# shamim-hussain/tgt

Hardware: AMD Instinct MI355X
Metric: graphs/sec training step, TGT-At 24L PCQM batch 256, 1/2/4/8 MI355X (higher is better)
Workload: dtype bf16

## Files before the change

tgt_amd/csrc/triplet_attention_bwd2.hip:

```cpp
#include <cstdlib>
#include "triplet_common.hpp"

namespace tgt {
namespace bwd2 {

typedef short s16x4 __attribute__((ext_vector_type(4)));
typedef __attribute__((address_space(3))) s16x4 lds_s16x4;

constexpr int HG = 8, D = 16, kThreads = 512;
constexpr int kRow = 256;
constexpr int kSlab = 32 * kRow;
constexpr int kSet = 4 * kSlab;
constexpr int kXch = 2 * 2048;
template <bool DMA> struct Lay {
#ifndef TGT_BWD2_DEPTH
#define TGT_BWD2_DEPTH 2
#endif
    static constexpr int kDepth = TGT_BWD2_DEPTH;
    static constexpr int kSets = DMA ? kDepth + 1 : 2;
    static constexpr int kOffXch = kSets * kSet;
    static constexpr int kOffPart = kOffXch + HG * kXch;
    static constexpr int kLds = kOffPart;
};
typedef __attribute__((address_space(3))) void lds_void;
#if TGT_LD_AUX == 2
#define TGT_BWD2_LD_POLICY " nt"
#else
#define TGT_BWD2_LD_POLICY ""
#endif

__device__ __forceinline__ int swz(int row) { return ((row & 7) << 1) | ((row >> 3) & 1); }
__device__ __forceinline__ int slab_off(int row, int cb) { return row * kRow + ((((cb >> 4) ^ swz(row)) & 15) << 4) + (cb & 15); }

__device__ __forceinline__ s16x4 tr_read(uint32_t addr) {
    return __builtin_amdgcn_ds_read_tr16_b64_v4i16(reinterpret_cast<lds_s16x4*>(addr));
}
template <typename T>
__device__ __forceinline__ frag_t<T> frag_of(s16x4 lo, s16x4 hi) {
    frag_t<T> f;
    __builtin_memcpy(&f, &lo, 8);
    __builtin_memcpy(reinterpret_cast<char*>(&f) + 8, &hi, 8);
    return f;
}
__device__ __forceinline__ f32x4 mma16(bf16x8 a, bf16x8 b, f32x4 c) { return __builtin_amdgcn_mfma_f32_16x16x32_bf16(a, b, c, 0, 0, 0); }
__device__ __forceinline__ f32x4 mma16(f16x8 a, f16x8 b, f32x4 c) { return __builtin_amdgcn_mfma_f32_16x16x32_f16(a, b, c, 0, 0, 0); }

template <typename T> struct Vec4;
template <> struct Vec4<bf16_t> { typedef __attribute__((ext_vector_type(4))) __bf16 type; };
template <> struct Vec4<f16_t> { typedef __attribute__((ext_vector_type(4))) _Float16 type; };
template <typename T>
__device__ __forceinline__ uint2 pack4(float a, float b, float c, float d) {
    typename Vec4<T>::type t;
    t[0] = from_f32<T>(a); t[1] = from_f32<T>(b); t[2] = from_f32<T>(c); t[3] = from_f32<T>(d);
    uint2 v;
    __builtin_memcpy(&v, &t, 8);
    return v;
}
template <typename T>
__device__ __forceinline__ uint2 frag_half(const frag_t<T>& f, int h) {
    uint2 v;
    __builtin_memcpy(&v, reinterpret_cast<const char*>(&f) + 8 * h, 8);
    return v;
}

template <typename T>
__device__ __forceinline__ void arm_load16(const ThirdArm& ta, int b, int dir, int g, int N, char* lds, int tid) {
    using A = ArmStage<T, HG, 1>;
    const int pitch = A::pitch(dir), mpitch = A::mpitch(dir);
    const char* eg = reinterpret_cast<const char*>(ta.eg);
    for (int idx = tid; idx < 32 * 32 * 2; idx += kThreads) {
        const int half = idx & 1, pr = idx >> 1, yy = pr & 31, xx = pr >> 5;
        uint4 v = make_uint4(0, 0, 0, 0);
        if (xx < N && yy < N && (half == 0 ? ta.biased : ta.gated))
            v = *reinterpret_cast<const uint4*>(eg + ((((int64_t)b * N + xx) * N + yy) * ta.ld + (half == 0 ? ta.e_off : ta.g_off) + g * HG) * 2);
        uint32_t* dst = reinterpret_cast<uint32_t*>(lds + xx * pitch + yy * A::kPairBytes + half * 16);
        dst[0] = v.x; dst[1] = v.y; dst[2] = v.z; dst[3] = v.w;
    }
    for (int idx = tid; idx < 32 * 32; idx += kThreads) {
        const int yy = idx & 31, xx = idx >> 5;
        float m = 0.f;
        if (xx < N && yy < N && ta.mask) m = ta.mask[((int64_t)b * N + xx) * N + yy];
        *reinterpret_cast<float*>(lds + A::kOffM + xx * mpitch + yy * 4) = m;
    }
}
template <typename T>
__device__ __forceinline__ void arm_store16(const ThirdArm& ta, void* d_eg, int b, int dir, int g, int N, const char* lds, int tid,
                                            float (&sums)[HG]) {
    using A = ArmStage<T, HG, 1>;
    const int pitch = A::pitch(dir);
    char* deg = reinterpret_cast<char*>(d_eg);
    static_assert(kThreads % 2 == 0, "a thread must own one piece (E or G)");
#pragma nounroll
    for (int idx = tid; idx < 32 * 32 * 2; idx += kThreads) {
        const int half = idx & 1, pr = idx >> 1, yy = pr & 31, xx = pr >> 5;
        if (xx < N && yy < N && (half == 0 ? ta.biased : ta.gated)) {
            const uint32_t* src = reinterpret_cast<const uint32_t*>(lds + xx * pitch + yy * A::kPairBytes + half * 16);
            const uint4 v = make_uint4(src[0], src[1], src[2], src[3]);
            *reinterpret_cast<uint4*>(deg + ((((int64_t)b * N + xx) * N + yy) * ta.ld + (half == 0 ? ta.e_off : ta.g_off) + g * HG) * 2) = v;
            T t[HG];
            __builtin_memcpy(t, &v, 16);
#pragma unroll
            for (int h = 0; h < HG; ++h) sums[h] += to_f32(t[h]);
        }
    }
}

__device__ __forceinline__ void zero_grad_rows(__amdgpu_buffer_rsrc_t r_grd, uint32_t wQ, uint32_t wK, uint32_t qo, uint32_t ko, uint32_t vo,
                                               uint32_t gQj, uint32_t gKj, int j0, int N) {
    const u32x4_t z = {0, 0, 0, 0};
    for (int j = j0; j < N; ++j) {
        __builtin_amdgcn_raw_buffer_store_b128(z, r_grd, (int)wQ, (int)(qo + (uint32_t)j * gQj), TGT_ST_AUX);
        __builtin_amdgcn_raw_buffer_store_b128(z, r_grd, (int)wK, (int)(ko + (uint32_t)j * gKj), TGT_ST_AUX);
        __builtin_amdgcn_raw_buffer_store_b128(z, r_grd, (int)wK, (int)(vo + (uint32_t)j * gKj), TGT_ST_AUX);
    }
}

template <typename T, bool CS, int FL, bool DMA, typename... NC>
__global__ void __launch_bounds__(kThreads, 2) __attribute__((amdgpu_waves_per_eu(2, 2))) tri_att_bwd2_kernel(const tgt_triplet_attention_args a, NC... nc) {
    constexpr bool RG = sizeof...(NC) > 0;
    const int32_t* node_counts = tri_counts_ptr(nc...);
    using F = frag_t<T>;
    constexpr int kOffXch = Lay<DMA>::kOffXch, kOffPart = Lay<DMA>::kOffPart;
    using G = TriGeo<T, D, HG>;
    extern __shared__ __attribute__((aligned(16))) char smem[];
    const uint32_t sbase = (uint32_t)(uintptr_t)smem;

    const int tid = threadIdx.x, lane = tid & 63, wave = tid >> 6;
    const int r = lane & 31, hi = lane >> 5;
    const int p16 = lane & 15, g16 = lane >> 4;
    const TriCtx c = tri_ctx<T, D, HG>(a, wave);
    const int N = c.N;
    const ThirdArm ta = tri_third_arm(a, c.dir);
    const bool biased = FL >= 0 ? (FL & TGT_TRI_BIASED) != 0 : ta.biased, gated = FL >= 0 ? (FL & TGT_TRI_GATED) != 0 : ta.gated;
    constexpr float kLog2e = 1.4426950408889634f;
    const float scale2 = a.scale * kLog2e;
#ifdef TGT_PROBES
    const int ablate = a._pad0;
#else
    constexpr int ablate = 0;
#endif

    const int64_t Nl = N;
    const int64_t ldq = a.ld_dqkv[c.dir] ? a.ld_dqkv[c.dir] : a.ld_qkv[c.dir];
    const int64_t lde = a.ld_deg[c.dir] ? a.ld_deg[c.dir] : a.ld_eg[c.dir];
    const uint32_t hch = (uint32_t)(c.g * HG * D * 2);
    const uint32_t lds_ = (uint32_t)(a.ld_qkv[c.dir] * 2), ldg_ = (uint32_t)(ldq * 2), ldo_ = (uint32_t)(a.ld_out * 2);
    const __amdgpu_buffer_rsrc_t r_src = graph_rsrc(a.qkv[c.dir], Nl * Nl * a.ld_qkv[c.dir] * 2, c.b);
    const __amdgpu_buffer_rsrc_t r_grd = graph_rsrc(a.d_qkv[c.dir], Nl * Nl * ldq * 2, c.b);
    const __amdgpu_buffer_rsrc_t r_do = graph_rsrc(a.d_out, Nl * Nl * a.ld_out * 2, c.b);
    const __amdgpu_buffer_rsrc_t r_src0 = __builtin_amdgcn_make_buffer_rsrc(const_cast<void*>(a.qkv[c.dir]), 0, 0, 0x00020000);
    const __amdgpu_buffer_rsrc_t r_do0 = __builtin_amdgcn_make_buffer_rsrc(const_cast<void*>(a.d_out), 0, 0, 0x00020000);
    const uint32_t qo = (uint32_t)(a.q_off[c.dir] * 2) + hch, ko = (uint32_t)(a.k_off[c.dir] * 2) + hch, vo = (uint32_t)(a.v_off[c.dir] * 2) + hch;
    const uint32_t oo = (uint32_t)(a.o_off[c.dir] * 2) + hch;
    const bool inward = c.dir == 0;
#ifdef TGT_PROBES
    const bool contig = (ablate & 8) != 0;
#else
    constexpr bool contig = false;
#endif
    const uint32_t sQr = contig ? lds_ : (uint32_t)N * lds_, sQj = contig ? (uint32_t)N * lds_ : lds_;
    const uint32_t sKr = (inward || contig) ? lds_ : (uint32_t)N * lds_, sKj = (inward || contig) ? (uint32_t)N * lds_ : lds_;
    const uint32_t gQr = contig ? ldg_ : (uint32_t)N * ldg_, gQj = contig ? (uint32_t)N * ldg_ : ldg_;
    const uint32_t gKr = (inward || contig) ? ldg_ : (uint32_t)N * ldg_, gKj = (inward || contig) ? (uint32_t)N * ldg_ : ldg_;
    const uint32_t oQr = contig ? ldo_ : (uint32_t)N * ldo_, oQj = contig ? (uint32_t)N * ldo_ : ldo_;
    ThirdArm dta = ta;
    dta.ld = lde;

    const int crow = tid >> 4, cslot = tid & 15;
    const uint32_t lslot16 = (uint32_t)((cslot ^ swz(crow)) & 15) * 16u;
    const uint32_t kOOB = 0x80000000u;
    const bool rowok = crow < N;
    const uint32_t vQ = rowok ? (uint32_t)crow * sQr + lslot16 : kOOB;
    const uint32_t vK = rowok ? (uint32_t)crow * sKr + lslot16 : kOOB;
    const uint32_t vO = rowok ? (uint32_t)crow * oQr + lslot16 : kOOB;
    const uint32_t wQ = rowok ? (uint32_t)crow * gQr + lslot16 : kOOB;
    const uint32_t wK = rowok ? (uint32_t)crow * gKr + lslot16 : kOOB;
    const int chunk = crow * kRow + cslot * 16;

    float* part = reinterpret_cast<float*>(smem + kOffXch);

    const bool dead = a.graph_scale && a.graph_scale[c.b] == 0.f;
    if (dead) {
        zero_grad_rows(r_grd, wQ, wK, qo, ko, vo, gQj, gKj, 0, N);
        const float zero16[16] = {0.f, 0.f, 0.f, 0.f, 0.f, 0.f, 0.f, 0.f, 0.f, 0.f, 0.f, 0.f, 0.f, 0.f, 0.f, 0.f};
        arm_stage_put_grad<T, HG, 1>(smem, c.dir, wave, r, hi, 0, zero16, zero16);
        __syncthreads();
        float unused[HG] = {0.f, 0.f, 0.f, 0.f, 0.f, 0.f, 0.f, 0.f};
        arm_store16<T>(dta, a.d_eg[c.dir], c.b, c.dir, c.g, N, smem, tid, unused);
        if constexpr (CS) {
            float* row = a.d_qkv_colsum[c.dir] + (int64_t)c.b * ldq + c.g * HG * D;
            if (tid < HG * D) {
                row[a.q_off[c.dir] + tid] = 0.f;
                row[a.k_off[c.dir] + tid] = 0.f;
                row[a.v_off[c.dir] + tid] = 0.f;
            }
            if (tid < 2 * HG && (biased || gated)) {
                float* erow = a.d_eg_colsum[c.dir] + (int64_t)c.b * lde;
                if (tid < HG) { if (biased) erow[a.e_off[c.dir] + c.g * HG + tid] = 0.f; }
                else if (gated) erow[a.g_off[c.dir] + c.g * HG + tid - HG] = 0.f;
            }
        }
        return;
    }

    const int n = tri_node_count<RG>(node_counts, c.b, N);
    if constexpr (RG) zero_grad_rows(r_grd, wQ, wK, qo, ko, vo, gQj, gKj, n, N);
    f32x2 biasM[8], gate[8], dE[8], dG[8];
    arm_load16<T>(ta, c.b, c.dir, c.g, N, smem, tid);
    __syncthreads();
    {
        float b16[16], g16[16];
        arm_stage_read<T, HG, 1, true>(ta, smem, c.dir, wave, N, r, hi, 0, 0, b16, g16);
#pragma unroll
        for (int q = 0; q < 16; ++q) {
            const float bl = b16[q] * kLog2e;
            b16[q] = (bl == -INFINITY && b16[q] != -INFINITY) ? -3.402823466e38f : bl;
        }
#pragma unroll
        for (int k = 0; k < 8; ++k) {
            biasM[k] = f32x2{b16[2 * k], b16[2 * k + 1]};
            gate[k] = f32x2{g16[2 * k], g16[2 * k + 1]};
            dE[k] = dG[k] = f32x2{0.f, 0.f};
        }
    }
    __syncthreads();

    const int hb = wave * 32;
    const uint32_t a_frag = (uint32_t)slab_off(r, hb + 16 * hi);
    const int c2 = p16 & 3, pr = p16 >> 2;
    const uint32_t a_kt0 = (uint32_t)slab_off(4 * hi + pr, hb + 8 * c2);
    const uint32_t a_kt1 = (uint32_t)slab_off(8 + 4 * hi + pr, hb + 8 * c2);
    const uint32_t a_qt = (uint32_t)slab_off(4 * g16 + pr, hb + 8 * c2);
    const uint32_t xw = (uint32_t)(kOffXch + wave * kXch + r * 32 + ((hi ^ ((r >> 2) & 3)) << 3));
    const uint32_t xr = (uint32_t)(kOffXch + wave * kXch + (4 * g16 + pr) * 32 + ((c2 ^ g16) << 3));
    const uint32_t w_q = (uint32_t)slab_off(r, hb + 8 * hi);
    const uint32_t w_kv = (uint32_t)slab_off(p16, hb + 8 * g16);

    f32x2 csq[4], csk[2], csv[2];
    if constexpr (CS) {
#pragma unroll
        for (int k = 0; k < 4; ++k) csq[k] = f32x2{0.f, 0.f};
        csk[0] = csk[1] = csv[0] = csv[1] = f32x2{0.f, 0.f};
    }

    auto issue = [&](u32x4_t (&pre)[4], int jj) {
        const bool live = jj < n && !(ablate & 1);
        const __amdgpu_buffer_rsrc_t rs = live ? r_src : r_src0, ro = live ? r_do : r_do0;
        pre[0] = __builtin_amdgcn_raw_buffer_load_b128(rs, (int)vQ, (int)(qo + (uint32_t)jj * sQj), TGT_LD_AUX);
        pre[1] = __builtin_amdgcn_raw_buffer_load_b128(ro, (int)vO, (int)(oo + (uint32_t)jj * oQj), TGT_LD_AUX);
        pre[2] = __builtin_amdgcn_raw_buffer_load_b128(rs, (int)vK, (int)(ko + (uint32_t)jj * sKj), TGT_LD_AUX);
        pre[3] = __builtin_amdgcn_raw_buffer_load_b128(rs, (int)vK, (int)(vo + (uint32_t)jj * sKj), TGT_LD_AUX);
    };
    auto commit = [&](const u32x4_t (&pre)[4], int set) {
        char* s = smem + set * kSet + chunk;
#pragma unroll
        for (int t = 0; t < 4; ++t) *reinterpret_cast<u32x4_t*>(s + t * kSlab) = pre[t];
    };
    const int wave_u = __builtin_amdgcn_readfirstlane(wave);
    const uint64_t src_base = (uint64_t)(uintptr_t)a.qkv[c.dir] + (uint64_t)c.b * (uint64_t)(Nl * Nl * a.ld_qkv[c.dir] * 2);
    const uint64_t do_base = (uint64_t)(uintptr_t)a.d_out + (uint64_t)c.b * (uint64_t)(Nl * Nl * a.ld_out * 2);
    const uint32_t src_bytes = (uint32_t)(Nl * Nl * a.ld_qkv[c.dir] * 2), do_bytes = (uint32_t)(Nl * Nl * a.ld_out * 2);
    auto dma = [&](int jj, int set) {
        const bool live = jj < n && !(ablate & 1);
        const u32x4_t rs = {(uint32_t)src_base, (uint32_t)(src_base >> 32) & 0xffffu, live ? src_bytes : 0u, 0x00020000u};
        const u32x4_t ro = {(uint32_t)do_base, (uint32_t)(do_base >> 32) & 0xffffu, live ? do_bytes : 0u, 0x00020000u};
        const uint32_t l0 = sbase + (uint32_t)(set * kSet + wave_u * 1024);
#define TGT_DMA16(LDSADDR, VOFF, RSRC, SOFF)                                                                                   \
        asm volatile("s_mov_b32 m0, %0\n\ts_nop 0\n\tbuffer_load_dwordx4 %1, %2, %3 offen" TGT_BWD2_LD_POLICY " lds"                                  \
                     :: "s"(LDSADDR), "v"(VOFF), "s"(RSRC), "s"(SOFF) : "memory")
        TGT_DMA16(l0, vQ, rs, qo + (uint32_t)jj * sQj);
        TGT_DMA16(l0 + kSlab, vO, ro, oo + (uint32_t)jj * oQj);
        TGT_DMA16(l0 + 2 * kSlab, vK, rs, ko + (uint32_t)jj * sKj);
        TGT_DMA16(l0 + 3 * kSlab, vK, rs, vo + (uint32_t)jj * sKj);
#undef TGT_DMA16
    };
    auto dummy_stores = [&]() {
        const u32x4_t z = {0, 0, 0, 0};
#pragma unroll
        for (int t = 0; t < 3; ++t) __builtin_amdgcn_raw_buffer_store_b128(z, r_grd, (int)kOOB, 16 * t, TGT_ST_AUX);
    };

    u32x4_t pre[4];
    if constexpr (DMA) {
        if (N < 32) {
            const u32x4_t z = {0, 0, 0, 0};
            for (int o = tid * 16; o < Lay<true>::kSets * kSet; o += kThreads * 16) *reinterpret_cast<u32x4_t*>(smem + o) = z;
            __syncthreads();
        }
        dma(0, 0);
#pragma unroll
        for (int d = 1; d < Lay<true>::kDepth; ++d) {
// ... 148 lines not shown
    }
    if constexpr (DMA) asm volatile("s_waitcnt vmcnt(0)" ::: "memory");
    __syncthreads();
    {
        float e16[16], g16v[16];
#pragma unroll
        for (int k = 0; k < 8; ++k) {
            f32x2 gg = dG[k];
            if (gated) gg *= gate[k] * (1.f - gate[k]);
            e16[2 * k] = dE[k].x; e16[2 * k + 1] = dE[k].y;
            g16v[2 * k] = gg.x; g16v[2 * k + 1] = gg.y;
        }
        arm_stage_put_grad<T, HG, 1>(smem, c.dir, wave, r, hi, 0, e16, g16v);
    }
    __syncthreads();
    {
        float pv[HG] = {0.f, 0.f, 0.f, 0.f, 0.f, 0.f, 0.f, 0.f};
        arm_store16<T>(dta, a.d_eg[c.dir], c.b, c.dir, c.g, N, smem, tid, pv);
        if constexpr (CS) {
#pragma unroll
            for (int h = 0; h < HG; ++h) part[tid * HG + h] = pv[h];
        }
    }
    if constexpr (CS) {
        float* row = a.d_qkv_colsum[c.dir] + (int64_t)c.b * ldq + c.g * HG * D + wave * D;
#pragma unroll
        for (int q = 0; q < 8; ++q) {
            const float v = group_sum<32>(q & 1 ? csq[q >> 1].y : csq[q >> 1].x);
            if (r == 0) row[a.q_off[c.dir] + (q & 3) + 8 * (q >> 2) + 4 * hi] = v;
        }
#pragma unroll
        for (int t = 0; t < 4; ++t) {
            const float vk = group_sum<16>(t & 1 ? csk[t >> 1].y : csk[t >> 1].x);
            const float vv = group_sum<16>(t & 1 ? csv[t >> 1].y : csv[t >> 1].x);
            if (p16 == 0) {
                row[a.k_off[c.dir] + 4 * g16 + t] = vk;
                row[a.v_off[c.dir] + 4 * g16 + t] = vv;
            }
        }
        __syncthreads();
        if (biased || gated) {
            constexpr int kVals = 2 * HG;
            if (tid < kVals) {
                float v = 0.f;
                for (int t = tid / HG; t < kThreads; t += 2) v += part[t * HG + tid % HG];
                float* erow = a.d_eg_colsum[c.dir] + (int64_t)c.b * lde;
                if (tid < HG) { if (biased) erow[a.e_off[c.dir] + c.g * HG + tid] = v; }
                else if (gated) erow[a.g_off[c.dir] + c.g * HG + tid - HG] = v;
            }
        }
    }
}

template <typename T, bool CS, int FL>
static int launch_one(const tgt_triplet_attention_args& a_in, const int32_t* nc, hipStream_t st) {
#ifdef TGT_PROBES
    tgt_triplet_attention_args a = a_in;
    a._pad0 = getenv("TGT_TRI_BWD_ABLATE") ? atoi(getenv("TGT_TRI_BWD_ABLATE")) : 0;
#else
    const tgt_triplet_attention_args& a = a_in;
#endif
    static const bool dma = !(getenv("TGT_TRI_BWD2_DMA") && atoi(getenv("TGT_TRI_BWD2_DMA")) == 0);
    const dim3 grid(a.B * 2 * (a.H / HG));
    if (dma) return (nc ? launch_lds<tri_att_bwd2_kernel<T, CS, FL, true, const int32_t*>>("tri_att_bwd2_kernel", grid, dim3(kThreads), Lay<true>::kLds, st, a, nc) : launch_lds<tri_att_bwd2_kernel<T, CS, FL, true>>("tri_att_bwd2_kernel", grid, dim3(kThreads), Lay<true>::kLds, st, a));
    return (nc ? launch_lds<tri_att_bwd2_kernel<T, CS, FL, false, const int32_t*>>("tri_att_bwd2_kernel", grid, dim3(kThreads), Lay<false>::kLds, st, a, nc) : launch_lds<tri_att_bwd2_kernel<T, CS, FL, false>>("tri_att_bwd2_kernel", grid, dim3(kThreads), Lay<false>::kLds, st, a));
}
template <typename T>
static int launch(const tgt_triplet_attention_args& a, const int32_t* nc, hipStream_t st) {
    constexpr int kBG = TGT_TRI_BIASED | TGT_TRI_GATED;
    const bool cs = a.d_qkv_colsum[0] != nullptr;
    if (cs && (a.flags & kBG) == kBG) return launch_one<T, true, kBG>(a, nc, st);
    if (cs) return launch_one<T, true, -1>(a, nc, st);
    return launch_one<T, false, -1>(a, nc, st);
}

}

bool tri_att_bwd2_eligible(const tgt_triplet_attention_args& a) {
    static const bool off = getenv("TGT_TRI_BWD2") && atoi(getenv("TGT_TRI_BWD2")) == 0;
    if (off || !((a.dtype == TGT_BF16 || a.dtype == TGT_F16) && a.D == 16 && a.N <= 32 && a.H % 8 == 0 && !(a.dropout_p > 0.f))) return false;
    if (a.flags & (TGT_TRI_BIASED | TGT_TRI_GATED))
        for (int dir = 0; dir < 2; ++dir) {
            const int64_t lde = a.ld_deg[dir] ? a.ld_deg[dir] : a.ld_eg[dir];
            if (a.ld_eg[dir] % 8 || lde % 8 || a.e_off[dir] % 8 || a.g_off[dir] % 8 || ((uintptr_t)a.eg[dir] | (uintptr_t)a.d_eg[dir]) % 16)
                return false;
        }
    return true;
}
int tri_att_bwd2_run(const tgt_triplet_attention_args& a, const int32_t* nc, hipStream_t st) {
    return a.dtype == TGT_BF16 ? bwd2::launch<bf16_t>(a, nc, st) : bwd2::launch<f16_t>(a, nc, st);
}

}
```

tgt_amd/csrc/triplet_attention_proj.hip:

```cpp
#include <cstdlib>
#include "triplet_common.hpp"

namespace tgt {

__device__ __forceinline__ f32x4 mma16x32(bf16x8 a, bf16x8 b, f32x4 c) { return __builtin_amdgcn_mfma_f32_16x16x32_bf16(a, b, c, 0, 0, 0); }
__device__ __forceinline__ f32x4 mma16x32(f16x8 a, f16x8 b, f32x4 c) { return __builtin_amdgcn_mfma_f32_16x16x32_f16(a, b, c, 0, 0, 0); }

namespace proj2 {
constexpr int kC = 256, kKS = 16, kRowBytes = kC * 2, kSlots = kRowBytes / 16;
constexpr int kXPitch = kRowBytes + 16;
constexpr int kXTile = 64 * kXPitch;
constexpr int kSlab = 32 * 8 * 16 * 2;
constexpr int kOffSets = 2 * kXTile, kSet = 3 * kSlab;
constexpr int kOffO = kOffSets + 2 * kSet, kOffBias = kOffO + 2 * kSlab;
constexpr int kLds = kOffBias + 8 * 48 * 4;
constexpr uint32_t kNone = 0xffffffffu;
__device__ __forceinline__ int xoff(int row, int slot) { return row * kXPitch + (slot << 4); }
}

__device__ __forceinline__ void zero_o_rows(__amdgpu_buffer_rsrc_t r_out, int tid, int N, uint32_t o_row, uint32_t o_base, uint32_t o_j, int j0) {
    const int srow = (tid & 511) >> 4, sslot = tid & 15;
    const uint32_t vo = (srow < N && tid >= 512) ? (uint32_t)srow * o_row + o_base + (uint32_t)sslot * 16u : proj2::kNone;
    for (int j = j0; j < N; ++j) {
        u32x4_t z = {0, 0, 0, 0};
        __builtin_amdgcn_raw_buffer_store_b128(z, r_out, (int)vo, (int)((uint32_t)j * o_j), TGT_ST_AUX);
    }
}

template <typename T, int DIR, bool STORE, bool RG>
__device__ __forceinline__ void proj2_walk(const tgt_triplet_attention_args& a, const int32_t* node_counts, const TriCtx& c,
                                           const T* x, const T* w, char* smem, int tid) {
    using namespace proj2;
    constexpr int D = 16, HG = 8;
    using G = TriGeo<T, D, HG>;
    using F = frag_t<T>;
    const int lane = tid & 63, wave = tid >> 6, r = lane & 31, hi = lane >> 5;
#ifdef TGT_PROBES
    const uint32_t ablate = a._pad1;
#else
    constexpr uint32_t ablate = 0;
#endif
    const bool attend = wave < 8;
    const int hw = wave & 7;
    const int N = c.N;
    char* xbuf = smem;
    char* sets = smem + kOffSets;
    char* oslab = smem + kOffO;
    const float* bias_w = reinterpret_cast<const float*>(smem + kOffBias) + hw * 48;

    const int64_t sz = sizeof(T), Nl = N;
    const __amdgpu_buffer_rsrc_t r_x = graph_rsrc(x, Nl * Nl * kRowBytes, c.b);
    const uint32_t hch = (uint32_t)(c.g * HG * D * sz), lds_ = (uint32_t)(a.ld_qkv[DIR] * sz), ldo_ = (uint32_t)(a.ld_out * sz);
    const __amdgpu_buffer_rsrc_t r_dst = graph_rsrc(a.qkv[DIR], Nl * Nl * a.ld_qkv[DIR] * sz, c.b);
    const __amdgpu_buffer_rsrc_t r_out = graph_rsrc(a.out, Nl * Nl * a.ld_out * sz, c.b);
    const uint32_t q_row = (uint32_t)N * lds_, q_j = lds_;
    const uint32_t kv_row = DIR == 0 ? lds_ : (uint32_t)N * lds_, kv_j = DIR == 0 ? (uint32_t)N * lds_ : lds_;
    const uint32_t o_row = (uint32_t)N * ldo_, o_j = ldo_;
    auto store_step = [&](int jq, bool qkv_live, int jo, bool o_live) {
        int t_ = tid;
        asm volatile("" : "+v"(t_));
        const int srow = (t_ & 511) >> 4, sslot = t_ & 15, shalf = t_ >> 9;
        const int s_lds = G::lds_off(srow, sslot);
        const bool row_ok = srow < N;
        const uint32_t c16 = (uint32_t)sslot * 16u + hch;
        if constexpr (!STORE) {
            const uint4 vb = *reinterpret_cast<const uint4*>(oslab + (jo & 1) * kSlab + s_lds);
            const uint32_t vo_o = (uint32_t)srow * o_row + (uint32_t)jo * o_j + (uint32_t)(a.o_off[DIR] * sz) + c16;
            u32x4_t db = {vb.x, vb.y, vb.z, vb.w};
            if (ablate & 2) return;
            __builtin_amdgcn_sched_barrier(0);
            __builtin_amdgcn_raw_buffer_store_b128(db, r_out, (int)((row_ok && o_live && shalf == 1) ? vo_o : kNone), 0, TGT_ST_AUX);
            __builtin_amdgcn_sched_barrier(0);
            return;
        }
        const char* set = sets + (jq & 1) * kSet;
        const uint4 va = *reinterpret_cast<const uint4*>(set + shalf * kSlab + s_lds);
        const uint4 vb = *reinterpret_cast<const uint4*>((shalf == 0 ? set + 2 * kSlab : oslab + (jo & 1) * kSlab) + s_lds);
        const uint32_t vo_a = (uint32_t)srow * (shalf == 0 ? q_row : kv_row) + (uint32_t)jq * (shalf == 0 ? q_j : kv_j) +
                              (uint32_t)((shalf == 0 ? a.q_off[DIR] : a.k_off[DIR]) * sz) + c16;
        const uint32_t vo_v = (uint32_t)srow * kv_row + (uint32_t)jq * kv_j + (uint32_t)(a.v_off[DIR] * sz) + c16;
        const uint32_t vo_o = (uint32_t)srow * o_row + (uint32_t)jo * o_j + (uint32_t)(a.o_off[DIR] * sz) + c16;
        u32x4_t da = {va.x, va.y, va.z, va.w}, db = {vb.x, vb.y, vb.z, vb.w};
        if (ablate & 2) return;
        __builtin_amdgcn_sched_barrier(0);
        __builtin_amdgcn_raw_buffer_store_b128(da, r_dst, (int)((row_ok && qkv_live) ? vo_a : kNone), 0, TGT_ST_AUX);
        __builtin_amdgcn_raw_buffer_store_b128(db, r_dst, (int)((row_ok && qkv_live && shalf == 0) ? vo_v : kNone), 0, TGT_ST_AUX);
        __builtin_amdgcn_raw_buffer_store_b128(db, r_out, (int)((row_ok && o_live && shalf == 1) ? vo_o : kNone), 0, TGT_ST_AUX);
        __builtin_amdgcn_sched_barrier(0);
    };

    const int n = tri_node_count<RG>(node_counts, c.b, N);
    if ((a.graph_scale && a.graph_scale[c.b] == 0.f) || (RG && n == 0)) {
        zero_o_rows(r_out, tid, N, o_row, (uint32_t)(a.o_off[DIR] * sz) + hch, o_j, 0);
        return;
    }

    const int l16 = lane & 15, l4 = lane >> 4;
#ifndef TGT_PROJ_PRIO
#define TGT_PROJ_PRIO 1
#endif
    if (TGT_PROJ_PRIO != 0 && __builtin_amdgcn_readfirstlane(wave) >= 8 == (TGT_PROJ_PRIO == 1)) __builtin_amdgcn_s_setprio(1);
    if (attend) {
        float biasM[16], gate[16];
        const ThirdArm ta = tri_third_arm(a, DIR);
        arm_stage_load<T, HG, 1>(ta, c.b, DIR, c.g, N, 0, smem, tid);
        __syncthreads();
        arm_stage_read<T, HG, 1, false>(ta, smem, DIR, hw, N, r, hi, 0, 0, biasM, gate);
        __syncthreads();
        constexpr int kXIt = DIR == 0 ? 4 : 2;
        uint32_t xvo[kXIt];
        int xlo[kXIt];
#pragma unroll
        for (int it = 0; it < kXIt; ++it) {
            const int cidx = it * 512 + tid, row = cidx >> 5, slot = cidx & 31;
            const int node = row & 31;
            xvo[it] = node < N ? (row < 32 ? (uint32_t)node * (uint32_t)N * kRowBytes : (uint32_t)node * kRowBytes) + (uint32_t)slot * 16u : kNone;
            xlo[it] = xoff(row, slot);
        }
        uint4 px[kXIt];
        auto x_issue = [&](int jx) {
            const bool live = jx < n && !(ablate & 1);
#pragma unroll
            for (int it = 0; it < kXIt; ++it) {
                const bool kvrows = DIR == 0 && it >= 2;
                const uint32_t so = live ? (uint32_t)jx * (kvrows ? (uint32_t)N * kRowBytes : (uint32_t)kRowBytes) : 0u;
                const u32x4_t v = __builtin_amdgcn_raw_buffer_load_b128(r_x, (int)(live ? xvo[it] : kNone), (int)so, 0);
                px[it] = make_uint4(v.x, v.y, v.z, v.w);
            }
        };
        auto x_commit = [&](int jx) {
            char* xt = xbuf + (jx & 1) * kXTile;
#pragma unroll
            for (int it = 0; it < kXIt; ++it) *reinterpret_cast<uint4*>(xt + xlo[it]) = px[it];
        };
        F ident_d[1];
        make_ident_d<T, 1>(ident_d, r, hi);
        x_issue(0);
        x_commit(0);
        x_issue(1);
        x_commit(1);
        __syncthreads();
        __syncthreads();
        if constexpr (STORE) store_step(0, true, 0, false);
        for (int j = 0; j < n; ++j) {
            x_issue(j + 2);
            asm volatile("" ::: "memory");
            if (!(ablate & 8)) {
                const char* set = sets + (j & 1) * kSet;
                F fq[1], fk[1], fv[1];
                read_frags<T, D, HG>(fq, set, hw, r, hi);
                read_frags<T, D, HG>(fk, set + kSlab, hw, r, hi);
                read_frags<T, D, HG>(fv, set + 2 * kSlab, hw, r, hi);
                f32x16 z0 = {0}, z1 = {0};
                f32x16 st = mma32(fk[0], fq[0], z0);
                f32x16 vt = mma32(fv[0], ident_d[0], z1);
                float mx = -INFINITY;
#pragma unroll
                for (int q = 0; q < 16; ++q) {
                    st[q] = st[q] * a.scale + biasM[q];
                    mx = fmaxf(mx, st[q]);
                }
                mx = fmaxf(mx, xhalf(mx));
                float sum = 0.f;
#pragma unroll
                for (int q = 0; q < 16; ++q) {
                    st[q] = fast_exp(st[q] - mx);
                    sum += st[q];
                }
                sum += xhalf(sum);
                const float inv = fast_rcp(sum);
#pragma unroll
                for (int q = 0; q < 16; ++q) st[q] = st[q] * inv * gate[q];
                f32x16 o = {0};
#pragma unroll
                for (int cc = 0; cc < 2; ++cc) o = mma32(pack_chunk<T>(vt, cc), pack_chunk<T>(st, cc), o);
                write_rows<T, D, HG>(oslab + (j & 1) * kSlab, o, hw, r, hi);
            }
            x_commit(j + 2);
            __syncthreads();
            if constexpr (STORE) store_step(j + 1, j + 1 < n, j, true);
        }
    } else {
        F wq[kKS / 2], wkv[kKS];
        {
            const T* rq = w + (int64_t)(a.q_off[DIR] + c.h * D + l16) * kC;
            const T* rkv = w + (int64_t)((r < 16 ? a.k_off[DIR] : a.v_off[DIR]) + c.h * D + (r & 15)) * kC;
#pragma unroll
            for (int s2 = 0; s2 < kKS / 2; ++s2) wq[s2] = load_frag<T>(rq + 32 * s2 + 8 * l4);
#pragma unroll
            for (int s2 = 0; s2 < kKS; ++s2) wkv[s2] = load_frag<T>(rkv + 16 * s2 + 8 * hi);
        }
        auto project = [&](int jn) {
            const char* xt = xbuf + (jn & 1) * kXTile;
            char* set = sets + (jn & 1) * kSet;
            constexpr int kv0 = DIR == 0 ? 32 : 0;
            {
                f32x16 kva;
#pragma unroll
                for (int q = 0; q < 16; ++q) kva[q] = bias_w[16 + acc_row(q, hi)];
#pragma unroll
                for (int s2 = 0; s2 < kKS; ++s2) {
                    const F xk = load_frag<T>(reinterpret_cast<const T*>(xt + xoff(kv0 + r, 2 * s2 + hi)));
                    kva = mma32(wkv[s2], xk, kva);
                    if ((s2 & 3) == 3) __builtin_amdgcn_sched_barrier(0);
                }
#pragma unroll
                for (int part = 0; part < 2; ++part)
#pragma unroll
                    for (int q = 0; q < 2; ++q) {
                        T tmp[4];
#pragma unroll
                        for (int t = 0; t < 4; ++t) tmp[t] = from_f32<T>(kva[8 * part + 4 * q + t]);
                        uint2 v;
                        __builtin_memcpy(&v, tmp, 8);
                        *reinterpret_cast<uint2*>(set + (1 + part) * kSlab + G::lds_elem(r, hw * D + 8 * q + 4 * hi)) = v;
                    }
            }
            __builtin_amdgcn_sched_barrier(0);
            {
                f32x4 q0, q1;
#pragma unroll
                for (int t = 0; t < 4; ++t) q0[t] = q1[t] = bias_w[4 * l4 + t];
#pragma unroll
                for (int s2 = 0; s2 < kKS / 2; ++s2) {
                    const F x0 = load_frag<T>(reinterpret_cast<const T*>(xt + xoff(l16, 4 * s2 + l4)));
                    const F x1 = load_frag<T>(reinterpret_cast<const T*>(xt + xoff(16 + l16, 4 * s2 + l4)));
                    q0 = mma16x32(wq[s2], x0, q0);
                    q1 = mma16x32(wq[s2], x1, q1);
                    if (s2 & 1) __builtin_amdgcn_sched_barrier(0);
                }
                T t0[4], t1[4];
#pragma unroll
                for (int t = 0; t < 4; ++t) { t0[t] = from_f32<T>(q0[t]); t1[t] = from_f32<T>(q1[t]); }
                uint2 v0, v1;
                __builtin_memcpy(&v0, t0, 8);
                __builtin_memcpy(&v1, t1, 8);
                *reinterpret_cast<uint2*>(set + G::lds_elem(l16, hw * D + 4 * l4)) = v0;
                *reinterpret_cast<uint2*>(set + G::lds_elem(16 + l16, hw * D + 4 * l4)) = v1;
            }
        };
        __syncthreads();
        __syncthreads();
        __syncthreads();
        project(0);
        __syncthreads();
        if constexpr (STORE) store_step(0, true, 0, false);
        for (int j = 0; j < n; ++j) {
            if (j + 1 < n && !(ablate & 4)) project(j + 1);
            __syncthreads();
            store_step(j + 1, j + 1 < n, j, true);
        }
    }
    if constexpr (RG) {
        int t_ = tid;
        asm volatile("" : "+v"(t_));
        zero_o_rows(r_out, t_, N, o_row, (uint32_t)(a.o_off[DIR] * sz) + hch, o_j, n);
    }
}

template <typename T, bool STORE, typename... NC>
__global__ void __launch_bounds__(1024, 4) tri_att_proj_fwd_kernel(const tgt_triplet_attention_args a, const T* x, const T* w, const T* bias,
                                                                   NC... nc) {
    constexpr bool RG = sizeof...(NC) > 0;
    const int32_t* node_counts = tri_counts_ptr(nc...);
    constexpr int D = 16, HG = 8;
    extern __shared__ __attribute__((aligned(16))) char smem[];
    const int tid = threadIdx.x, lane = tid & 63, wave = tid >> 6;
    const TriCtx c = tri_ctx<T, D, HG>(a, wave & 7);
    const int dir = c.dir;
    if (wave >= 8 && lane < 48) {
        const int part = lane >> 4, d = lane & 15;
        const int off = part == 0 ? a.q_off[dir] : (part == 1 ? a.k_off[dir] : a.v_off[dir]);
        reinterpret_cast<float*>(smem + proj2::kOffBias)[(wave & 7) * 48 + lane] = to_f32(bias[off + c.h * D + d]);
    }
    if (dir == 0) proj2_walk<T, 0, STORE, RG>(a, node_counts, c, x, w, smem, tid);
    else proj2_walk<T, 1, STORE, RG>(a, node_counts, c, x, w, smem, tid);
}

template <typename T>
static int launch_proj(const tgt_triplet_attention_args& a, const int32_t* nc, const void* x, const void* w, const void* bias, hipStream_t st) {
    const int grid = a.B * 2 * (a.H / 8);
    static_assert(ArmStage<T, 8, 1>::kBytes <= proj2::kOffO, "arm stage must fit the aliased area");
#ifdef TGT_PROBES
    static const int ablate = getenv("TGT_PROJ_ABLATE") ? atoi(getenv("TGT_PROJ_ABLATE")) : 0;
    tgt_triplet_attention_args aa = a;
    aa._pad1 = (uint32_t)ablate;
#else
    const tgt_triplet_attention_args& aa = a;
#endif
    const T *xp = reinterpret_cast<const T*>(x), *wp = reinterpret_cast<const T*>(w), *bp = reinterpret_cast<const T*>(bias);
    const dim3 g(grid), blk(1024);
    if (a.flags & TGT_TRI_NO_QKV_STORE)
        return nc ? launch_lds<tri_att_proj_fwd_kernel<T, false, const int32_t*>>("tri_att_proj_fwd_kernel", g, blk, proj2::kLds, st, aa, xp, wp, bp, nc)
                  : launch_lds<tri_att_proj_fwd_kernel<T, false>>("tri_att_proj_fwd_kernel", g, blk, proj2::kLds, st, aa, xp, wp, bp);
    return nc ? launch_lds<tri_att_proj_fwd_kernel<T, true, const int32_t*>>("tri_att_proj_fwd_kernel", g, blk, proj2::kLds, st, aa, xp, wp, bp, nc)
              : launch_lds<tri_att_proj_fwd_kernel<T, true>>("tri_att_proj_fwd_kernel", g, blk, proj2::kLds, st, aa, xp, wp, bp);
}

int triplet_attention_proj_supported(const tgt_triplet_attention_args* a, int C) {
    return a && a->dropout_p == 0.f && a->N <= 32 && a->D == 16 && a->H % 8 == 0 && (a->dtype == TGT_BF16 || a->dtype == TGT_F16) &&
           C == 256;
}

int triplet_attention_proj_run(const tgt_triplet_attention_args* a, const int32_t* nc, const void* x, int C, const void* w,
                               const void* bias, hipStream_t st) {
    if (!a || !x || !w || !bias) return set_error(TGT_ERR_INVALID, "projected triplet attention: null argument");
    if (a->B < 0 || a->N < 0 || a->H <= 0) return set_error(TGT_ERR_INVALID, "projected triplet attention: bad sizes");
    if (a->B == 0 || a->N == 0) return TGT_OK;
    if (!triplet_attention_proj_supported(a, C))
        return set_error(TGT_ERR_UNSUPPORTED,
                         "projected triplet attention needs N <= 32, D = 16, H %% 8 == 0, a 16-bit dtype, C = 256 and no attention dropout "
                         "(got N=%d D=%d H=%d dtype=%d C=%d)", a->N, a->D, a->H, a->dtype, C);
    const bool store = !(a->flags & TGT_TRI_NO_QKV_STORE);
    for (int dir = 0; dir < 2; ++dir) {
        if ((store && !a->qkv[dir]) || !a->out || !a->mask) return set_error(TGT_ERR_INVALID, "projected triplet attention: null tensor");
        if (store && ((a->ld_qkv[dir] * 2) % 16 || (a->q_off[dir] * 2) % 16 || (a->k_off[dir] * 2) % 16 || (a->v_off[dir] * 2) % 16 ||
                      ((uintptr_t)a->qkv[dir] % 16)))
            return set_error(TGT_ERR_INVALID, "projected triplet attention: rows/offsets must be 16-byte aligned");
        if ((a->ld_out * 2) % 16 || (a->o_off[dir] * 2) % 16 || ((uintptr_t)a->out % 16))
            return set_error(TGT_ERR_INVALID, "projected triplet attention: rows/offsets must be 16-byte aligned");
        if ((a->flags & (TGT_TRI_BIASED | TGT_TRI_GATED)) && !a->eg[dir]) return set_error(TGT_ERR_INVALID, "projected triplet attention: eg missing");
    }
    if (((uintptr_t)x | (uintptr_t)w) % 16) return set_error(TGT_ERR_INVALID, "projected triplet attention: x / w must be 16-byte aligned");
    return a->dtype == TGT_BF16 ? launch_proj<bf16_t>(*a, nc, x, w, bias, st) : launch_proj<f16_t>(*a, nc, x, w, bias, st);
}

}
```

tgt_amd/csrc/triplet_common.hpp:

```cpp
#pragma once
#include "common.hpp"

namespace tgt {

template <typename T, int D, int HG>
struct TriGeo {
    static constexpr int kThreads = HG * 64;
    static constexpr int kRowBytes = HG * D * (int)sizeof(T);
    static constexpr int kSlots = kRowBytes / 16;
    static constexpr int kSlabBytes = 32 * kRowBytes;
    static constexpr int kChunks = 32 * kSlots;
    static constexpr int kIters = (kChunks + kThreads - 1) / kThreads;
    static constexpr int kRowsPerBankRow = kRowBytes >= 256 ? 1 : 256 / kRowBytes;
    static constexpr int kSwzMask = (kSlots < 16 ? kSlots : 16) - 1;
    static constexpr int kDC = (D + 15) / 16;
    static_assert(kRowBytes % 16 == 0, "row piece must be a multiple of 16 bytes");
    static_assert(D % 8 == 0 && D <= 32, "D in {8,16,24,32}");

    __device__ static __forceinline__ int lds_off(int row, int slot) {
        const int f = (row / kRowsPerBankRow) & kSwzMask;
        return row * kRowBytes + ((slot ^ f) << 4);
    }
    __device__ static __forceinline__ int lds_elem(int row, int col) {
        const int bo = col * (int)sizeof(T);
// ... 201 lines not shown
}


struct ThirdArm {
    const void* eg;
    int64_t ld;
    int e_off, g_off;
    const float* mask;
    bool biased, gated;
};

template <typename T, bool PAD_COLS_NEG_INF>
__device__ __forceinline__ void load_third_arm(const ThirdArm& ta, int b, int dir, int h, int N, int r, int hi,
                                               float (&biasM)[16], float (&gate)[16], int i0 = 0, int k0 = 0) {
    const T* eg = reinterpret_cast<const T*>(ta.eg);
#pragma unroll
    for (int q = 0; q < 16; ++q) {
        const int k = k0 + acc_row(q, hi), i = i0 + r;
        const bool valid = i < N && k < N;
        const int x = dir == 0 ? i : k, y = dir == 0 ? k : i;
        const int64_t idx = ((int64_t)b * N + x) * N + y;
        const float m = (valid && ta.mask) ? ta.mask[idx] : 0.f;
        float e = 0.f, gl = 0.f;
        if (valid && ta.biased) e = to_f32(eg[idx * ta.ld + ta.e_off + h]);
        if (valid && ta.gated) gl = to_f32(eg[idx * ta.ld + ta.g_off + h]);
        biasM[q] = (k < N && (!PAD_COLS_NEG_INF || i < N)) ? e + m : -INFINITY;
        gate[q] = valid ? (ta.gated ? fast_sigmoid(gl + m) : 1.f) : 0.f;
    }
}

template <typename T>
__device__ __forceinline__ void store_third_arm_grad(const ThirdArm& ta, void* d_eg, int b, int dir, int h, int N,
                                                     int r, int hi, const float (&dE)[16], const float (&dG)[16],
                                                     int i0 = 0, int k0 = 0) {
    if (!(ta.biased || ta.gated)) return;
    T* deg = reinterpret_cast<T*>(d_eg);
#pragma unroll
    for (int q = 0; q < 16; ++q) {
        const int k = k0 + acc_row(q, hi), i = i0 + r;
        if (i < N && k < N) {
            const int x = dir == 0 ? i : k, y = dir == 0 ? k : i;
            const int64_t idx = ((int64_t)b * N + x) * N + y;
            if (ta.biased) deg[idx * ta.ld + ta.e_off + h] = from_f32<T>(dE[q]);
            if (ta.gated) deg[idx * ta.ld + ta.g_off + h] = from_f32<T>(dG[q]);
        }
    }
}

template <typename T, int HG, int NT>
struct ArmStage {
    static constexpr int kVals = 2 * HG;
    static constexpr int kPairBytes = kVals * (int)sizeof(T);
    static constexpr int kOffM = ((32 * NT * 32 * kPairBytes + 4 * 32 * NT + 15) / 16) * 16;
    static constexpr int kBytes = kOffM + 32 * NT * 32 * 4 + 4 * 32 * NT;
    __device__ static __forceinline__ int nx(int dir) { return dir == 0 ? 32 : 32 * NT; }
    __device__ static __forceinline__ int ny(int dir) { return dir == 0 ? 32 * NT : 32; }
    __device__ static __forceinline__ int pitch(int dir) { return ny(dir) * kPairBytes + 4; }
    __device__ static __forceinline__ int mpitch(int dir) { return ny(dir) * 4 + 4; }
};

template <typename T, int HG, int NT>
__device__ __forceinline__ void arm_stage_load(const ThirdArm& ta, int b, int dir, int g, int N, int i0, char* lds,
                                               int tid, int k0 = 0) {
    using A = ArmStage<T, HG, NT>;
    const int nx = A::nx(dir), ny = A::ny(dir), x0 = dir == 0 ? i0 : k0, y0 = dir == 0 ? k0 : i0;
    const int pitch = A::pitch(dir), mpitch = A::mpitch(dir);
    const T* eg = reinterpret_cast<const T*>(ta.eg);
    for (int idx = tid; idx < nx * ny * A::kVals; idx += HG * 64) {
        const int v = idx % A::kVals, p = idx / A::kVals, yy = p % ny, xx = p / ny;
        const int x = x0 + xx, y = y0 + yy;
        T val = from_f32<T>(0.f);
        if (x < N && y < N) {
            const bool is_e = v < HG;
            if (is_e ? ta.biased : ta.gated)
                val = eg[(((int64_t)b * N + x) * N + y) * ta.ld + (is_e ? ta.e_off + g * HG + v : ta.g_off + g * HG + v - HG)];
        }
        *reinterpret_cast<T*>(lds + xx * pitch + yy * A::kPairBytes + v * (int)sizeof(T)) = val;
    }
    for (int idx = tid; idx < nx * ny; idx += HG * 64) {
        const int yy = idx % ny, xx = idx / ny, x = x0 + xx, y = y0 + yy;
        float m = 0.f;
        if (x < N && y < N && ta.mask) m = ta.mask[((int64_t)b * N + x) * N + y];
        *reinterpret_cast<float*>(lds + A::kOffM + xx * mpitch + yy * 4) = m;
    }
}

template <typename T, int HG, int NT, bool PAD_COLS_NEG_INF>
__device__ __forceinline__ void arm_stage_read(const ThirdArm& ta, const char* lds, int dir, int hh, int N, int r, int hi,
                                               int i0, int kt, float (&biasM)[16], float (&gate)[16], int k0 = 0) {
    using A = ArmStage<T, HG, NT>;
    const int pitch = A::pitch(dir), mpitch = A::mpitch(dir);
#pragma unroll
    for (int q = 0; q < 16; ++q) {
        const int kl = 32 * kt + acc_row(q, hi), k = k0 + kl, i = i0 + r;
        const bool valid = i < N && k < N;
        const int xx = dir == 0 ? r : kl, yy = dir == 0 ? kl : r;
        const char* pp = lds + xx * pitch + yy * A::kPairBytes;
        const float e = to_f32(*reinterpret_cast<const T*>(pp + hh * (int)sizeof(T)));
        const float gl = to_f32(*reinterpret_cast<const T*>(pp + (HG + hh) * (int)sizeof(T)));
        const float m = *reinterpret_cast<const float*>(lds + A::kOffM + xx * mpitch + yy * 4);
        biasM[q] = (k < N && (!PAD_COLS_NEG_INF || i < N)) ? e + m : -INFINITY;
        gate[q] = valid ? (ta.gated ? fast_sigmoid(gl + m) : 1.f) : 0.f;
    }
}

template <typename T, int HG, int NT>
__device__ __forceinline__ void arm_stage_put_grad(char* lds, int dir, int hh, int r, int hi, int kt,
                                                   const float (&dE)[16], const float (&dG)[16]) {
    using A = ArmStage<T, HG, NT>;
    const int pitch = A::pitch(dir);
#pragma unroll
    for (int q = 0; q < 16; ++q) {
        const int kl = 32 * kt + acc_row(q, hi);
        const int xx = dir == 0 ? r : kl, yy = dir == 0 ? kl : r;
        char* pp = lds + xx * pitch + yy * A::kPairBytes;
        *reinterpret_cast<T*>(pp + hh * (int)sizeof(T)) = from_f32<T>(dE[q]);
        *reinterpret_cast<T*>(pp + (HG + hh) * (int)sizeof(T)) = from_f32<T>(dG[q]);
    }
}

template <typename T, int HG, int NT>
__device__ __forceinline__ float arm_stage_store_grad(const ThirdArm& ta, void* d_eg, int b, int dir, int g, int N,
                                                      int i0, const char* lds, int tid, int k0 = 0) {
    using A = ArmStage<T, HG, NT>;
    static_assert((HG * 64) % A::kVals == 0, "a thread must own one E/G column");
    float part = 0.f;
    if (!(ta.biased || ta.gated)) return part;
    const int nx = A::nx(dir), ny = A::ny(dir), x0 = dir == 0 ? i0 : k0, y0 = dir == 0 ? k0 : i0;
    const int pitch = A::pitch(dir);
    T* deg = reinterpret_cast<T*>(d_eg);
#pragma nounroll
    for (int idx = tid; idx < nx * ny * A::kVals; idx += HG * 64) {
        const int v = idx % A::kVals, p = idx / A::kVals, yy = p % ny, xx = p / ny;
        const int x = x0 + xx, y = y0 + yy;
        const bool is_e = v < HG;
        if (x < N && y < N && (is_e ? ta.biased : ta.gated)) {
            const T val = *reinterpret_cast<const T*>(lds + xx * pitch + yy * A::kPairBytes + v * (int)sizeof(T));
            deg[(((int64_t)b * N + x) * N + y) * ta.ld + (is_e ? ta.e_off + g * HG + v : ta.g_off + g * HG + v - HG)] = val;
            part += to_f32(val);
        }
    }
    return part;
}

template <int NT>
__device__ __forceinline__ void tile_softmax(float (&p)[NT][16]) {
    float mx = -INFINITY;
#pragma unroll
    for (int kt = 0; kt < NT; ++kt)
#pragma unroll
        for (int q = 0; q < 16; ++q) mx = fmaxf(mx, p[kt][q]);
    mx = fmaxf(mx, xhalf(mx));
    if (mx == -INFINITY) mx = 0.f;
    float sum = 0.f;
#pragma unroll
    for (int kt = 0; kt < NT; ++kt)
#pragma unroll
        for (int q = 0; q < 16; ++q) {
            p[kt][q] = fast_exp(p[kt][q] - mx);
            sum += p[kt][q];
        }
    sum += xhalf(sum);
    const float inv = sum > 0.f ? fast_rcp(sum) : 0.f;
#pragma unroll
    for (int kt = 0; kt < NT; ++kt)
#pragma unroll
// ... 121 lines not shown
```

Baseline: 3242.

## Batch third-arm edge loads via buffer loads and overlap with x prefetch

Adds an ArmBatch helper that issues all edge/gate/mask loads for a head group up front with raw buffer loads, using out-of-range offsets for padding, then commits them to LDS afterwards. The projected forward kernel now issues these loads together with the first two x-tile prefetches before staging, so their latencies overlap. The bwd2 kernel uses the same batched path, with a fallback when alignment does not hold, which lets the eligibility check drop the eg pointer alignment requirement. The proj kernel also drops the node-count template variant in favour of a runtime check, which cuts instantiations but adds a branch and an always-run zero-rows tail, and the batched loads raise register pressure.

Result: no change. 3271 (median of 6 runs) (+0.9%).

```diff
diff --git a/tgt_amd/csrc/triplet_attention_bwd2.hip b/tgt_amd/csrc/triplet_attention_bwd2.hip
--- a/tgt_amd/csrc/triplet_attention_bwd2.hip
+++ b/tgt_amd/csrc/triplet_attention_bwd2.hip
@@ -63,26 +63,6 @@
     return v;
 }
 
-template <typename T>
-__device__ __forceinline__ void arm_load16(const ThirdArm& ta, int b, int dir, int g, int N, char* lds, int tid) {
-    using A = ArmStage<T, HG, 1>;
-    const int pitch = A::pitch(dir), mpitch = A::mpitch(dir);
-    const char* eg = reinterpret_cast<const char*>(ta.eg);
-    for (int idx = tid; idx < 32 * 32 * 2; idx += kThreads) {
-        const int half = idx & 1, pr = idx >> 1, yy = pr & 31, xx = pr >> 5;
-        uint4 v = make_uint4(0, 0, 0, 0);
-        if (xx < N && yy < N && (half == 0 ? ta.biased : ta.gated))
-            v = *reinterpret_cast<const uint4*>(eg + ((((int64_t)b * N + xx) * N + yy) * ta.ld + (half == 0 ? ta.e_off : ta.g_off) + g * HG) * 2);
-        uint32_t* dst = reinterpret_cast<uint32_t*>(lds + xx * pitch + yy * A::kPairBytes + half * 16);
-        dst[0] = v.x; dst[1] = v.y; dst[2] = v.z; dst[3] = v.w;
-    }
-    for (int idx = tid; idx < 32 * 32; idx += kThreads) {
-        const int yy = idx & 31, xx = idx >> 5;
-        float m = 0.f;
-        if (xx < N && yy < N && ta.mask) m = ta.mask[((int64_t)b * N + xx) * N + yy];
-        *reinterpret_cast<float*>(lds + A::kOffM + xx * mpitch + yy * 4) = m;
-    }
-}
 template <typename T>
 __device__ __forceinline__ void arm_store16(const ThirdArm& ta, void* d_eg, int b, int dir, int g, int N, const char* lds, int tid,
                                             float (&sums)[HG]) {
@@ -206,7 +186,13 @@
     const int n = tri_node_count<RG>(node_counts, c.b, N);
     if constexpr (RG) zero_grad_rows(r_grd, wQ, wK, qo, ko, vo, gQj, gKj, n, N);
     f32x2 biasM[8], gate[8], dE[8], dG[8];
-    arm_load16<T>(ta, c.b, c.dir, c.g, N, smem, tid);
+    if (arm_batch_ok<T, HG>(ta, c.g, N)) {
+        ArmBatch<T, HG, 1, kThreads> ab;
+        arm_batch_issue(ab, ta, c.b, c.dir, c.g, N, 0, tid);
+        arm_batch_commit(ab, c.dir, smem, tid);
+    } else {
+        arm_stage_load<T, HG, 1>(ta, c.b, c.dir, c.g, N, 0, smem, tid);
+    }
     __syncthreads();
     {
         float b16[16], g16[16];
@@ -521,7 +507,7 @@
     if (a.flags & (TGT_TRI_BIASED | TGT_TRI_GATED))
         for (int dir = 0; dir < 2; ++dir) {
             const int64_t lde = a.ld_deg[dir] ? a.ld_deg[dir] : a.ld_eg[dir];
-            if (a.ld_eg[dir] % 8 || lde % 8 || a.e_off[dir] % 8 || a.g_off[dir] % 8 || ((uintptr_t)a.eg[dir] | (uintptr_t)a.d_eg[dir]) % 16)
+            if (a.ld_eg[dir] % 8 || lde % 8 || a.e_off[dir] % 8 || a.g_off[dir] % 8 || (uintptr_t)a.d_eg[dir] % 16)
                 return false;
         }
     return true;
diff --git a/tgt_amd/csrc/triplet_attention_proj.hip b/tgt_amd/csrc/triplet_attention_proj.hip
--- a/tgt_amd/csrc/triplet_attention_proj.hip
+++ b/tgt_amd/csrc/triplet_attention_proj.hip
@@ -27,7 +27,7 @@
     }
 }
 
-template <typename T, int DIR, bool STORE, bool RG>
+template <typename T, int DIR, bool STORE>
 __device__ __forceinline__ void proj2_walk(const tgt_triplet_attention_args& a, const int32_t* node_counts, const TriCtx& c,
                                            const T* x, const T* w, char* smem, int tid) {
     using namespace proj2;
@@ -89,8 +89,8 @@
         __builtin_amdgcn_sched_barrier(0);
     };
 
-    const int n = tri_node_count<RG>(node_counts, c.b, N);
-    if ((a.graph_scale && a.graph_scale[c.b] == 0.f) || (RG && n == 0)) {
+    const int n = node_counts ? tri_node_count<true>(node_counts, c.b, N) : N;
+    if ((a.graph_scale && a.graph_scale[c.b] == 0.f) || n == 0) {
         zero_o_rows(r_out, tid, N, o_row, (uint32_t)(a.o_off[DIR] * sz) + hch, o_j, 0);
         return;
     }
@@ -103,10 +103,9 @@
     if (attend) {
         float biasM[16], gate[16];
         const ThirdArm ta = tri_third_arm(a, DIR);
-        arm_stage_load<T, HG, 1>(ta, c.b, DIR, c.g, N, 0, smem, tid);
-        __syncthreads();
-        arm_stage_read<T, HG, 1, false>(ta, smem, DIR, hw, N, r, hi, 0, 0, biasM, gate);
-        __syncthreads();
+        const bool batched = arm_batch_ok<T, HG>(ta, c.g, N);
+        ArmBatch<T, HG, 1, 512> ab;
+        if (batched) arm_batch_issue(ab, ta, c.b, DIR, c.g, N, 0, tid);
         constexpr int kXIt = DIR == 0 ? 4 : 2;
         uint32_t xvo[kXIt];
         int xlo[kXIt];
@@ -117,8 +116,8 @@
             xvo[it] = node < N ? (row < 32 ? (uint32_t)node * (uint32_t)N * kRowBytes : (uint32_t)node * kRowBytes) + (uint32_t)slot * 16u : kNone;
             xlo[it] = xoff(row, slot);
         }
-        uint4 px[kXIt];
-        auto x_issue = [&](int jx) {
+        uint4 px[kXIt], px1[kXIt];
+        auto x_issue = [&](uint4 (&px)[kXIt], int jx) {
             const bool live = jx < n && !(ablate & 1);
 #pragma unroll
             for (int it = 0; it < kXIt; ++it) {
@@ -128,22 +127,27 @@
                 px[it] = make_uint4(v.x, v.y, v.z, v.w);
             }
         };
-        auto x_commit = [&](int jx) {
+        auto x_commit = [&](const uint4 (&px)[kXIt], int jx) {
             char* xt = xbuf + (jx & 1) * kXTile;
 #pragma unroll
             for (int it = 0; it < kXIt; ++it) *reinterpret_cast<uint4*>(xt + xlo[it]) = px[it];
         };
         F ident_d[1];
         make_ident_d<T, 1>(ident_d, r, hi);
-        x_issue(0);
-        x_commit(0);
-        x_issue(1);
-        x_commit(1);
+        x_issue(px, 0);
+        x_issue(px1, 1);
+        if (batched) arm_batch_commit(ab, DIR, smem, tid);
+        else arm_stage_load<T, HG, 1>(ta, c.b, DIR, c.g, N, 0, smem, tid);
+        __syncthreads();
+        arm_stage_read<T, HG, 1, false>(ta, smem, DIR, hw, N, r, hi, 0, 0, biasM, gate);
+        __syncthreads();
+        x_commit(px, 0);
+        x_commit(px1, 1);
         __syncthreads();
         __syncthreads();
         if constexpr (STORE) store_step(0, true, 0, false);
         for (int j = 0; j < n; ++j) {
-            x_issue(j + 2);
+            x_issue(px, j + 2);
             asm volatile("" ::: "memory");
             if (!(ablate & 8)) {
                 const char* set = sets + (j & 1) * kSet;
@@ -176,7 +180,7 @@
                 for (int cc = 0; cc < 2; ++cc) o = mma32(pack_chunk<T>(vt, cc), pack_chunk<T>(st, cc), o);
                 write_rows<T, D, HG>(oslab + (j & 1) * kSlab, o, hw, r, hi);
             }
-            x_commit(j + 2);
+            x_commit(px, j + 2);
             __syncthreads();
             if constexpr (STORE) store_step(j + 1, j + 1 < n, j, true);
         }
@@ -251,18 +255,16 @@
             store_step(j + 1, j + 1 < n, j, true);
         }
     }
-    if constexpr (RG) {
+    {
         int t_ = tid;
         asm volatile("" : "+v"(t_));
         zero_o_rows(r_out, t_, N, o_row, (uint32_t)(a.o_off[DIR] * sz) + hch, o_j, n);
     }
 }
 
-template <typename T, bool STORE, typename... NC>
+template <typename T, bool STORE>
 __global__ void __launch_bounds__(1024, 4) tri_att_proj_fwd_kernel(const tgt_triplet_attention_args a, const T* x, const T* w, const T* bias,
-                                                                   NC... nc) {
-    constexpr bool RG = sizeof...(NC) > 0;
-    const int32_t* node_counts = tri_counts_ptr(nc...);
+                                                                   const int32_t* node_counts) {
     constexpr int D = 16, HG = 8;
     extern __shared__ __attribute__((aligned(16))) char smem[];
     const int tid = threadIdx.x, lane = tid & 63, wave = tid >> 6;
@@ -273,8 +275,8 @@
         const int off = part == 0 ? a.q_off[dir] : (part == 1 ? a.k_off[dir] : a.v_off[dir]);
         reinterpret_cast<float*>(smem + proj2::kOffBias)[(wave & 7) * 48 + lane] = to_f32(bias[off + c.h * D + d]);
     }
-    if (dir == 0) proj2_walk<T, 0, STORE, RG>(a, node_counts, c, x, w, smem, tid);
-    else proj2_walk<T, 1, STORE, RG>(a, node_counts, c, x, w, smem, tid);
+    if (dir == 0) proj2_walk<T, 0, STORE>(a, node_counts, c, x, w, smem, tid);
+    else proj2_walk<T, 1, STORE>(a, node_counts, c, x, w, smem, tid);
 }
 
 template <typename T>
@@ -291,10 +293,8 @@
     const T *xp = reinterpret_cast<const T*>(x), *wp = reinterpret_cast<const T*>(w), *bp = reinterpret_cast<const T*>(bias);
     const dim3 g(grid), blk(1024);
     if (a.flags & TGT_TRI_NO_QKV_STORE)
-        return nc ? launch_lds<tri_att_proj_fwd_kernel<T, false, const int32_t*>>("tri_att_proj_fwd_kernel", g, blk, proj2::kLds, st, aa, xp, wp, bp, nc)
-                  : launch_lds<tri_att_proj_fwd_kernel<T, false>>("tri_att_proj_fwd_kernel", g, blk, proj2::kLds, st, aa, xp, wp, bp);
-    return nc ? launch_lds<tri_att_proj_fwd_kernel<T, true, const int32_t*>>("tri_att_proj_fwd_kernel", g, blk, proj2::kLds, st, aa, xp, wp, bp, nc)
-              : launch_lds<tri_att_proj_fwd_kernel<T, true>>("tri_att_proj_fwd_kernel", g, blk, proj2::kLds, st, aa, xp, wp, bp);
+        return launch_lds<tri_att_proj_fwd_kernel<T, false>>("tri_att_proj_fwd_kernel", g, blk, proj2::kLds, st, aa, xp, wp, bp, nc);
+    return launch_lds<tri_att_proj_fwd_kernel<T, true>>("tri_att_proj_fwd_kernel", g, blk, proj2::kLds, st, aa, xp, wp, bp, nc);
 }
 
 int triplet_attention_proj_supported(const tgt_triplet_attention_args* a, int C) {
diff --git a/tgt_amd/csrc/triplet_common.hpp b/tgt_amd/csrc/triplet_common.hpp
--- a/tgt_amd/csrc/triplet_common.hpp
+++ b/tgt_amd/csrc/triplet_common.hpp
@@ -307,6 +307,65 @@
         float m = 0.f;
         if (x < N && y < N && ta.mask) m = ta.mask[((int64_t)b * N + x) * N + y];
         *reinterpret_cast<float*>(lds + A::kOffM + xx * mpitch + yy * 4) = m;
+    }
+}
+
+template <typename T, int HG, int NT, int THREADS>
+struct ArmBatch {
+    static_assert(HG * (int)sizeof(T) == 16, "E (G) of the head group must be one 16-byte piece");
+    static_assert((32 * NT * 32) % THREADS == 0, "whole trips");
+    static constexpr int kPieces = 32 * NT * 32 * 2 / THREADS, kMask = 32 * NT * 32 / THREADS;
+    u32x4_t piece[kPieces];
+    uint32_t mask[kMask];
+};
+template <typename T, int HG>
+__device__ __forceinline__ bool arm_batch_ok(const ThirdArm& ta, int g, int N) {
+    if (!(ta.biased || ta.gated)) return true;
+    const int64_t sz = sizeof(T);
+    const uint64_t eb = ta.biased ? (uint64_t)((ta.e_off + g * HG) * sz) : 0, gb = ta.gated ? (uint64_t)((ta.g_off + g * HG) * sz) : 0;
+    return (((uint64_t)(uintptr_t)ta.eg | (uint64_t)(ta.ld * sz) | eb | gb) & 15) == 0 && ta.ld > 0 &&
+           (int64_t)N * N * ta.ld * sz < ((int64_t)1 << 31);
+}
+template <typename T, int HG, int NT, int THREADS>
+__device__ __forceinline__ void arm_batch_issue(ArmBatch<T, HG, NT, THREADS>& ab, const ThirdArm& ta, int b, int dir, int g, int N,
+                                                int i0, int tid, int k0 = 0) {
+    using A = ArmStage<T, HG, NT>;
+    constexpr uint32_t kNone = 0xffffffffu;
+    const int64_t sz = sizeof(T), Nl = N;
+    const int ny = A::ny(dir), x0 = dir == 0 ? i0 : k0, y0 = dir == 0 ? k0 : i0;
+    const __amdgpu_buffer_rsrc_t r_eg = graph_rsrc(ta.eg, (ta.biased || ta.gated) ? Nl * Nl * ta.ld * sz : 0, b);
+    const __amdgpu_buffer_rsrc_t r_m = graph_rsrc(ta.mask, ta.mask ? Nl * Nl * 4 : 0, b);
+    const uint32_t ldb = (uint32_t)(ta.ld * sz);
+    const uint32_t eb = ta.biased ? (uint32_t)((ta.e_off + g * HG) * sz) : kNone, gb = ta.gated ? (uint32_t)((ta.g_off + g * HG) * sz) : kNone;
+#pragma unroll
+    for (int it = 0; it < ab.kPieces; ++it) {
+        const int idx = it * THREADS + tid, half = idx & 1, pr = idx >> 1, yy = pr % ny, xx = pr / ny;
+        const int x = x0 + xx, y = y0 + yy;
+        const uint32_t col = half == 0 ? eb : gb;
+        const uint32_t vo = ((uint32_t)(x * N + y) * ldb + col) | (0u - (uint32_t)!(x < N && y < N && col != kNone));
+        ab.piece[it] = __builtin_amdgcn_raw_buffer_load_b128(r_eg, (int)vo, 0, 0);
+    }
+#pragma unroll
+    for (int it = 0; it < ab.kMask; ++it) {
+        const int idx = it * THREADS + tid, yy = idx % ny, xx = idx / ny, x = x0 + xx, y = y0 + yy;
+        const uint32_t vo = ((uint32_t)(x * N + y) * 4u) | (0u - (uint32_t)!(x < N && y < N));
+        ab.mask[it] = __builtin_amdgcn_raw_buffer_load_b32(r_m, (int)vo, 0, 0);
+    }
+}
+template <typename T, int HG, int NT, int THREADS>
+__device__ __forceinline__ void arm_batch_commit(const ArmBatch<T, HG, NT, THREADS>& ab, int dir, char* lds, int tid) {
+    using A = ArmStage<T, HG, NT>;
+    const int ny = A::ny(dir), pitch = A::pitch(dir), mpitch = A::mpitch(dir);
+#pragma unroll
+    for (int it = 0; it < ab.kPieces; ++it) {
+        const int idx = it * THREADS + tid, half = idx & 1, pr = idx >> 1, yy = pr % ny, xx = pr / ny;
+        uint32_t* dst = reinterpret_cast<uint32_t*>(lds + xx * pitch + yy * A::kPairBytes + half * 16);
+        dst[0] = ab.piece[it].x; dst[1] = ab.piece[it].y; dst[2] = ab.piece[it].z; dst[3] = ab.piece[it].w;
+    }
+#pragma unroll
+    for (int it = 0; it < ab.kMask; ++it) {
+        const int idx = it * THREADS + tid, yy = idx % ny, xx = idx / ny;
+        *reinterpret_cast<uint32_t*>(lds + A::kOffM + xx * mpitch + yy * 4) = ab.mask[it];
     }
 }
 
```
